# akamiru/bce

Hardware: AMD Instinct MI355X
Metric: MB/s compressed (higher is better)
Workload: dtype u8/u32 integer

## Files before the change

### bce_amd/csrc/host_coder.cpp

```cpp
#include "host_coder.h"

#include "bce_core.h"

#include <stdio.h>
#include <stdlib.h>
#include <string.h>

#include <chrono>
#include <thread>

namespace bce {

const uint8_t kDefaultConfig[9][32] = {
    {0, 0, 5, 5, 5, 4, 4, 4, 4, 4, 4, 4, 4, 4, 4, 4, 4, 4, 4, 4, 4, 4, 4, 4, 4, 4, 4, 4, 4, 4, 4, 0},
    {0, 0, 5, 5, 5, 4, 4, 4, 4, 4, 4, 4, 4, 4, 4, 4, 4, 4, 4, 4, 4, 4, 4, 4, 4, 4, 4, 4, 4, 4, 4, 0},
    {0, 0, 5, 5, 5, 4, 4, 4, 4, 4, 4, 4, 4, 4, 4, 4, 4, 4, 4, 4, 4, 4, 4, 4, 4, 4, 4, 3, 3, 3, 3, 0},
    {0, 0, 5, 5, 5, 4, 4, 4, 4, 4, 4, 4, 4, 4, 4, 4, 4, 4, 4, 4, 4, 4, 3, 3, 3, 3, 3, 3, 3, 3, 3, 0},
    {0, 0, 5, 5, 4, 4, 4, 4, 4, 4, 4, 4, 3, 3, 3, 3, 3, 3, 3, 3, 3, 3, 3, 3, 3, 3, 3, 3, 3, 3, 3, 0},
    {0, 0, 5, 5, 4, 4, 4, 4, 4, 4, 4, 4, 3, 3, 3, 3, 3, 3, 3, 3, 3, 3, 3, 3, 3, 3, 3, 3, 3, 3, 3, 0},
    {0, 0, 5, 4, 4, 4, 4, 4, 4, 3, 3, 3, 3, 3, 3, 3, 3, 3, 3, 3, 3, 3, 3, 3, 3, 3, 3, 3, 3, 3, 3, 0},
    {0, 0, 4, 4, 4, 4, 3, 3, 3, 3, 3, 3, 3, 3, 3, 3, 3, 3, 3, 3, 3, 3, 3, 3, 3, 2, 2, 2, 2, 2, 2, 0},
    {0, 0, 0, 0, 0, 0, 0, 0, 0, 0, 0, 0, 0, 0, 0, 0, 0, 0, 0, 0, 0, 0, 0, 0, 0, 0, 0, 0, 0, 0, 0, 0}};

void RangeCoder::setv(uint32_t s) {
  while (s) { uniform(s & 1, 3); s >>= 1; }
  uniform(2, 3);
}

void RangeCoder::preamble(const uint8_t row[32]) {
  uint32_t last = 0;
  for (int b = 0; b < 32; ++b) {
    const uint32_t bit = row[b];
    uniform(bit != last, 2);
    if (bit != last) uniform(bit, 6);
    last = bit;
  }
}

void RangeCoder::flush() {
  while (!((h_ ^ l_) >> 48)) {
    data_.push_back((uint16_t)(h_ >> 48));
    l_ = (l_ << 16) + 0x0000;
    h_ = (h_ << 16) + 0xFFFF;
  }
  const uint32_t bits = (uint32_t)__builtin_clzll(l_ ^ h_) + 1;
  data_.push_back((uint16_t)((h_ >> (64 - bits)) << (16 - bits)));
}

void HostCoder::begin(const uint8_t config[9][32], const uint32_t C[8], uint32_t n) {
  drain();
  failed_.store(false);
  for (int i = 0; i < 8; ++i) {
    w_[i].busy = 0; w_[i].nsym = 0; w_[i].idle = 0; w_[i].started = false;
    plane[i] = RangeCoder();
    plane[i].preamble(config[i]);
    plane[i].uniform(C[i], n + 1);
  }
}

const Recip *recip_table() {
  static const std::vector<Recip> tab = [] {
    std::vector<Recip> t(kRecipMax);
    t[0] = t[1] = Recip{0, -1, 0};
    for (uint32_t d = 2; d < kRecipMax; ++d) {
      uint32_t L = 0;
      while ((2ull << L) <= d) ++L;
      if ((d & (d - 1)) == 0) { t[d] = Recip{1ull << (64 - L), -1, 0}; continue; }
      const unsigned __int128 two_s = (unsigned __int128)1 << (64 + L);
      const uint64_t m_dn = (uint64_t)(two_s / d);
      const uint64_t e_dn = (uint64_t)(two_s - (unsigned __int128)m_dn * d);
      const uint64_t e_up = d - e_dn;
      if (e_up <= (1ull << L)) t[d] = Recip{m_dn + 1, -1, L};
      else t[d] = Recip{m_dn, 0, L};
    }
    return t;
  }();
  return tab.data();
}

uint64_t bce_test_div_recip(uint64_t x, uint32_t d) {
  return x == ~0ull ? x / d : div_recip1(x + 1, recip_table()[d]);
}

void RangeCoder::encode_run(const uint64_t *out, uint64_t begin, uint64_t end) {
  const Recip *rt = recip_table();
  uint64_t l = l_, R = h_ - l_ + 1;
  uint16_t stage[64];
  uint32_t ns = 0;
#define BCE_EMIT(v)                                                                                       \
  do {                                                                                                    \
    stage[ns++] = (uint16_t)(v);                                                                          \
    if (__builtin_expect(ns == 64, 0)) { data_.insert(data_.end(), stage, stage + 64); ns = 0; }          \
  } while (0)
#define BCE_STEP(cum, freq, total)                                                                        \
  do {                                                                                                    \
    const uint32_t t_ = (total);                                                                          \
    if (__builtin_expect(R - 1 < t_, 0)) {                                                  \
      for (int i_ = 0; i_ < 4; ++i_) BCE_EMIT(l >> (48 - 16 * i_));                                       \
      l = 0; R = 0;                                                                                       \
    }                                                                                                     \
    const uint64_t step_ =                                                                                \
        (__builtin_expect(R == 0, 0) || t_ >= kRecipMax) ? (R - 1) / t_ : div_recip1(R, rt[t_]);          \
    l += step_ * (cum);                                                                         \
    R = step_ * (freq);                                                \
    while (__builtin_expect(!(((l + R - 1) ^ l) >> 48), 0)) {                     \
      BCE_EMIT((l + R - 1) >> 48);                                                                        \
      l <<= 16;                                                                                           \
      R <<= 16;                                                             \
    }                                                                                                     \
  } while (0)
#define BCE_BIT(bit)                                                                                      \
  do {                                                                                                    \
    if (__builtin_expect(R - 1 < 2u, 0)) {                                                  \
      for (int i_ = 0; i_ < 4; ++i_) BCE_EMIT(l >> (48 - 16 * i_));                                       \
      l = 0; R = 0;                                                                                       \
    }                                                                                                     \
    const uint64_t step_ = (R - 1) >> 1;                                                                  \
    l += step_ & (0ull - (uint64_t)(bit));                                                                \
    R = step_;                                                                                            \
    while (__builtin_expect(!(((l + R - 1) ^ l) >> 48), 0)) {                                             \
      BCE_EMIT((l + R - 1) >> 48);                                                                        \
      l <<= 16;                                                                                           \
      R <<= 16;                                                                                           \
    }                                                                                                     \
  } while (0)
  for (uint64_t i = begin; i < end; ++i) {
    const uint64_t o = out[i];
    uint32_t es = out_esc_sentinel(o);
    if (__builtin_expect(es != 1u, 0))
      for (; es > 1u; es >>= 1) BCE_BIT(es & 1u);
    BCE_STEP(out_cum(o), out_freq(o), out_total(o));
  }
#undef BCE_BIT
#undef BCE_STEP
#undef BCE_EMIT
  data_.insert(data_.end(), stage, stage + ns);
  l_ = l; h_ = l + R - 1;
}

void HostCoder::consume(int p, const SymRun *runs, size_t nruns, const uint64_t *out) {
  RangeCoder &rc = plane[p];
  for (size_t r = 0; r < nruns; ++r) rc.encode_run(out, runs[r].start, runs[r].start + runs[r].count);
}

HostCoder::HostCoder() {
  try {
    for (int p = 0; p < 8; ++p) w_[p].th = std::thread([this, p]() { run(p); });
  } catch (...) {
    stop_threads();
    throw;
  }
}

void HostCoder::stop_threads() {
  for (int p = 0; p < 8; ++p) {
    { std::lock_guard<std::mutex> g(w_[p].mu); w_[p].stop = true; }
    w_[p].cv.notify_all();
  }
  for (int p = 0; p < 8; ++p) if (w_[p].th.joinable()) w_[p].th.join();
}

HostCoder::~HostCoder() { stop_threads(); }

void HostCoder::run(int p) {
  Worker &w = w_[p];
  for (;;) {
    CoderBatch *b = nullptr;
    double wait_s = 0;
    {
      std::unique_lock<std::mutex> lk(w.mu);
      const bool dry = w.q.empty();
      const auto tw = std::chrono::steady_clock::now();
      w.cv.wait(lk, [&] { return w.stop || !w.q.empty(); });
      if (w.q.empty()) return;
      b = w.q.front();
      w.q.pop_front();
      wait_s = dry ? std::chrono::duration<double>(std::chrono::steady_clock::now() - tw).count() : 0.0;
    }
    const auto t0 = std::chrono::steady_clock::now();
    try {
      if (b->wait_ready) {
        b->wait_ready();
        wait_s += std::chrono::duration<double>(std::chrono::steady_clock::now() - t0).count();
      }
      if (!failed_.load(std::memory_order_relaxed) && ((plane_mask >> p) & 1u)) {
        consume(p, b->runs[p].data(), b->runs[p].size(), b->out);
        for (const SymRun &r : b->runs[p]) w.nsym += r.count;
      }
    } catch (...) {
      failed_.store(true);
    }
    const double dt = std::chrono::duration<double>(std::chrono::steady_clock::now() - t0).count();
    {
      std::lock_guard<std::mutex> g(done_mu_);
      w.busy += dt;
      if (w.started) w.idle += wait_s;
      w.started = true;
      b->pending.fetch_sub(1);
      ++completed_;
    }
    done_cv_.notify_all();
  }
}

void HostCoder::submit(CoderBatch *b) {
  b->pending.store(8);
  { std::lock_guard<std::mutex> g(done_mu_); submitted_ += 8; }
  for (int p = 0; p < 8; ++p) {
    { std::lock_guard<std::mutex> g(w_[p].mu); w_[p].q.push_back(b); }
    w_[p].cv.notify_one();
  }
}

void HostCoder::wait(CoderBatch *b) {
  std::unique_lock<std::mutex> lk(done_mu_);
  done_cv_.wait(lk, [&] { return b->pending.load() == 0; });
}

void HostCoder::drain() {
  std::unique_lock<std::mutex> lk(done_mu_);
  done_cv_.wait(lk, [&] { return completed_ == submitted_; });
}

double HostCoder::busy_seconds() {
  std::lock_guard<std::mutex> g(done_mu_);
  double m = 0;
  for (int p = 0; p < 8; ++p) m = w_[p].busy > m ? w_[p].busy : m;
  return m;
}

double HostCoder::idle_seconds(int p) {
  std::lock_guard<std::mutex> g(done_mu_);
  return w_[p].idle;
}

void HostCoder::finish(const uint8_t config[9][32], uint32_t n, uint32_t offset) {
  if (getenv("BCE_HIP_CODER_DEBUG"))
    for (int p = 0; p < 8; ++p) fprintf(stderr, "coder %d: busy %.1f ms, %llu symbols, %zu words\n", p, w_[p].busy * 1e3, (unsigned long long)w_[p].nsym, plane[p].data().size());
  for (int i = 0; i < 8; ++i) plane[i].flush();
  rebuild_header(config, n, offset);
}

void HostCoder::rebuild_header(const uint8_t config[9][32], uint32_t n, uint32_t offset) {
  unsigned size = 0u;
  for (int i = 0; i < 8; ++i) size += (unsigned)plane[i].data().size();
  RangeCoder mainc;
  mainc.preamble(config[8]);
  mainc.setv(n);
  mainc.uniform(offset, n + 1);
  mainc.setv(size);
  int s = (int)size;
  for (int i = 0; i < 7; ++i) {
    mainc.uniform((uint32_t)plane[i].data().size(), (uint32_t)s + 1);
    s -= (int)plane[i].data().size();
  }
  mainc.flush();
  header_ = mainc.data();
}

size_t HostCoder::archive_words() const {
  size_t w = 1 + header_.size();
  for (int i = 0; i < 8; ++i) w += plane[i].data().size();
  return w;
}

void HostCoder::assemble(uint16_t *dst) const {
  *dst++ = (uint16_t)header_.size();
  memcpy(dst, header_.data(), header_.size() * 2);
  dst += header_.size();
  uint16_t *at[8];
  for (int i = 0; i < 8; ++i) { at[i] = dst; dst += plane[i].data().size(); }
  size_t total = 0;
  for (int i = 0; i < 8; ++i) total += plane[i].data().size();
  if (total < (1u << 20)) {
    for (int i = 0; i < 8; ++i) memcpy(at[i], plane[i].data().data(), plane[i].data().size() * 2);
    return;
  }
  std::thread th[8];
  int started = 0;
  try {
    for (; started < 8; ++started) {
      const int i = started;
      th[i] = std::thread([this, i, &at] { memcpy(at[i], plane[i].data().data(), plane[i].data().size() * 2); });
    }
  } catch (...) {
  }
  for (int i = started; i < 8; ++i) memcpy(at[i], plane[i].data().data(), plane[i].data().size() * 2);
  for (int i = 0; i < started; ++i) th[i].join();
}

void HostCoder::finish(const uint8_t config[9][32], uint32_t n, uint32_t offset, std::vector<uint16_t> &archive) {
  finish(config, n, offset);
  archive.resize(archive_words());
  assemble(archive.data());
}

}
```

### bce_amd/csrc/host_coder.h

```cpp
#pragma once
#include <stddef.h>
#include <stdint.h>

#include <atomic>
#include <condition_variable>
#include <deque>
#include <functional>
#include <mutex>
#include <thread>
#include <vector>

namespace bce {

class alignas(128) RangeCoder {
 public:
  RangeCoder() : l_(0), h_(~0ull) {}
  inline void encode(uint32_t cum, uint32_t freq, uint32_t total) {
    if (__builtin_expect(h_ - l_ < total, 0)) {
      for (int i = 0; i < 4; ++i) data_.push_back((uint16_t)(l_ >> (48 - 16 * i)));
      l_ = 0; h_ = ~0ull;
    }
    const uint64_t step = (h_ - l_) / total;
    l_ += step * cum;
    h_ = l_ + step * freq - 1;
    while (!((h_ ^ l_) >> 48)) {
      data_.push_back((uint16_t)(h_ >> 48));
      l_ = (l_ << 16) + 0x0000;
      h_ = (h_ << 16) + 0xFFFF;
    }
  }
  inline void uniform(uint32_t s, uint32_t k) { encode(s, 1, k); }
  void setv(uint32_t s);
  void preamble(const uint8_t row[32]);
  void flush();
  const std::vector<uint16_t> &data() const { return data_; }
  std::vector<uint16_t> &data() { return data_; }
  void encode_run(const uint64_t *out, uint64_t begin, uint64_t end);

 private:
  uint64_t l_, h_;
  std::vector<uint16_t> data_;
};

struct SymRun { uint64_t start; uint32_t count; uint32_t round; };

struct CoderBatch {
  const uint64_t *out = nullptr;
  std::function<void()> wait_ready;
  std::vector<SymRun> runs[8];
  std::atomic<int> pending{0};
};

struct HostCoder {
  RangeCoder plane[8];
  uint32_t plane_mask = 0xFFu;
  void set_stream(int p, const uint16_t *words, size_t n) { plane[p].data().assign(words, words + n); }
  void rebuild_header(const uint8_t config[9][32], uint32_t n, uint32_t offset);
  HostCoder();
  ~HostCoder();
  void begin(const uint8_t config[9][32], const uint32_t C[8], uint32_t n);
  void consume(int p, const SymRun *runs, size_t nruns, const uint64_t *out);
  void submit(CoderBatch *b);
  void wait(CoderBatch *b);
  void drain();
  void finish(const uint8_t config[9][32], uint32_t n, uint32_t offset);
  size_t archive_words() const;
  void assemble(uint16_t *dst) const;
  void finish(const uint8_t config[9][32], uint32_t n, uint32_t offset, std::vector<uint16_t> &archive);
  double busy_seconds();
  double idle_seconds(int p);
  bool failed() const { return failed_.load(); }

 private:
  struct Worker {
    std::thread th;
    std::mutex mu;
    std::condition_variable cv;
    std::deque<CoderBatch *> q;
    double busy = 0, idle = 0;
    bool started = false;
    uint64_t nsym = 0;
    bool stop = false;
  };
  Worker w_[8];
  std::mutex done_mu_;
  std::condition_variable done_cv_;
  std::vector<uint16_t> header_;
  uint64_t submitted_ = 0, completed_ = 0;
  std::atomic<bool> failed_{false};
  void run(int p);
  void stop_threads();
};

struct Recip { uint64_t m; int32_t am1; uint32_t sh; };
constexpr uint32_t kRecipMax = 8192;
const Recip *recip_table();
inline uint64_t div_recip1(uint64_t x1, const Recip &r) {
  return (uint64_t)(((unsigned __int128)r.m * (x1 + (uint64_t)(int64_t)r.am1)) >> 64) >> r.sh;
}
inline uint64_t div_small(uint64_t x, uint32_t d, const Recip *rt) {
  return (x == ~0ull || d >= kRecipMax) ? x / d : div_recip1(x + 1, rt[d]);
}

extern const uint8_t kDefaultConfig[9][32];
uint64_t bce_test_div_recip(uint64_t x, uint32_t d);

}
```

Before: 922.0.

## Reuse persistent coder workers for archive assembly copy and align hot encode loop

Archive assembly no longer spawns eight fresh std::threads per call. It hands each persistent coder worker an equal byte slice of the concatenated streams to memcpy, with a small copy flag and a pending counter guarded by the existing done mutex. This spreads the copy evenly across threads instead of one thread per plane, and it removes thread creation cost. The encode_run hot loop is also placed in its own 64-byte-aligned text section, with an optional padding knob. Debug timing instrumentation for the coder tail is added too, at the cost of extra clock reads and more synchronisation state.

```diff
diff --git a/bce_amd/csrc/host_coder.cpp b/bce_amd/csrc/host_coder.cpp
--- a/bce_amd/csrc/host_coder.cpp
+++ b/bce_amd/csrc/host_coder.cpp
@@ -6,6 +6,7 @@
 #include <stdlib.h>
 #include <string.h>
 
+#include <algorithm>
 #include <chrono>
 #include <thread>
 
@@ -47,8 +48,12 @@
   data_.push_back((uint16_t)((h_ >> (64 - bits)) << (16 - bits)));
 }
 
+static double steady_s() { return std::chrono::duration<double>(std::chrono::steady_clock::now().time_since_epoch()).count(); }
+
 void HostCoder::begin(const uint8_t config[9][32], const uint32_t C[8], uint32_t n) {
+  const double t0 = steady_s();
   drain();
+  std::lock_guard<std::mutex> copying(copy_mu_);
   failed_.store(false);
   for (int i = 0; i < 8; ++i) {
     w_[i].busy = 0; w_[i].nsym = 0; w_[i].idle = 0; w_[i].started = false;
@@ -56,6 +61,7 @@
     plane[i].preamble(config[i]);
     plane[i].uniform(C[i], n + 1);
   }
+  t_begin_s_ = steady_s() - t0;
 }
 
 const Recip *recip_table() {
@@ -82,7 +88,18 @@
   return x == ~0ull ? x / d : div_recip1(x + 1, recip_table()[d]);
 }
 
-void RangeCoder::encode_run(const uint64_t *out, uint64_t begin, uint64_t end) {
+#ifdef BCE_CODER_UNPLACED
+#define BCE_HOT_LOOP
+#elif defined(BCE_CODER_PAD)
+#define BCE_STR2(x) #x
+#define BCE_STR(x) BCE_STR2(x)
+__asm__(".pushsection .text.bce_encode_run,\"ax\",@progbits\n.balign 64\n.skip " BCE_STR(BCE_CODER_PAD) ", 0xcc\n.popsection");
+#define BCE_HOT_LOOP __attribute__((section(".text.bce_encode_run"), aligned(16)))
+#else
+#define BCE_HOT_LOOP __attribute__((section(".text.bce_encode_run"), aligned(64)))
+#endif
+
+BCE_HOT_LOOP void RangeCoder::encode_run(const uint64_t *out, uint64_t begin, uint64_t end) {
   const Recip *rt = recip_table();
   uint64_t l = l_, R = h_ - l_ + 1;
   uint16_t stage[64];
@@ -167,15 +184,28 @@
   for (;;) {
     CoderBatch *b = nullptr;
     double wait_s = 0;
+    bool copy = false;
     {
       std::unique_lock<std::mutex> lk(w.mu);
       const bool dry = w.q.empty();
       const auto tw = std::chrono::steady_clock::now();
-      w.cv.wait(lk, [&] { return w.stop || !w.q.empty(); });
-      if (w.q.empty()) return;
-      b = w.q.front();
-      w.q.pop_front();
-      wait_s = dry ? std::chrono::duration<double>(std::chrono::steady_clock::now() - tw).count() : 0.0;
+      w.cv.wait(lk, [&] { return w.stop || w.copy || !w.q.empty(); });
+      if (!w.q.empty()) {
+        b = w.q.front();
+        w.q.pop_front();
+        wait_s = dry ? std::chrono::duration<double>(std::chrono::steady_clock::now() - tw).count() : 0.0;
+      } else if (w.copy) {
+        w.copy = false;
+        copy = true;
+      } else {
+        return;
+      }
+    }
+    if (copy) {
+      copy_streams(copy_dst_, copy_words_ * (size_t)p / 8, copy_words_ * (size_t)(p + 1) / 8);
+      { std::lock_guard<std::mutex> g(done_mu_); --copy_pending_; }
+      done_cv_.notify_all();
+      continue;
     }
     const auto t0 = std::chrono::steady_clock::now();
     try {
@@ -190,9 +220,11 @@
     } catch (...) {
       failed_.store(true);
     }
-    const double dt = std::chrono::duration<double>(std::chrono::steady_clock::now() - t0).count();
+    const auto t1 = std::chrono::steady_clock::now();
+    const double dt = std::chrono::duration<double>(t1 - t0).count();
     {
       std::lock_guard<std::mutex> g(done_mu_);
+      t_batch_done_ = std::max(t_batch_done_, std::chrono::duration<double>(t1.time_since_epoch()).count());
       w.busy += dt;
       if (w.started) w.idle += wait_s;
       w.started = true;
@@ -220,6 +252,7 @@
 void HostCoder::drain() {
   std::unique_lock<std::mutex> lk(done_mu_);
   done_cv_.wait(lk, [&] { return completed_ == submitted_; });
+  t_drained_ = steady_s();
 }
 
 double HostCoder::busy_seconds() {
@@ -237,8 +270,10 @@
 void HostCoder::finish(const uint8_t config[9][32], uint32_t n, uint32_t offset) {
   if (getenv("BCE_HIP_CODER_DEBUG"))
     for (int p = 0; p < 8; ++p) fprintf(stderr, "coder %d: busy %.1f ms, %llu symbols, %zu words\n", p, w_[p].busy * 1e3, (unsigned long long)w_[p].nsym, plane[p].data().size());
+  t_finish0_ = steady_s();
   for (int i = 0; i < 8; ++i) plane[i].flush();
   rebuild_header(config, n, offset);
+  t_finish1_ = steady_s();
 }
 
 void HostCoder::rebuild_header(const uint8_t config[9][32], uint32_t n, uint32_t offset) {
@@ -264,29 +299,52 @@
   return w;
 }
 
-void HostCoder::assemble(uint16_t *dst) const {
+void HostCoder::copy_streams(uint16_t *dst, size_t from, size_t to) const {
+  size_t at = 0;
+  for (int i = 0; i < 8 && at < to; ++i) {
+    const std::vector<uint16_t> &d = plane[i].data();
+    const size_t lo = from > at ? from : at, hi = to < at + d.size() ? to : at + d.size();
+    if (lo < hi) memcpy(dst + lo, d.data() + (lo - at), (hi - lo) * 2);
+    at += d.size();
+  }
+}
+
+bool HostCoder::copy_by_threads(uint16_t *dst, size_t words) {
+  if (failed()) return false;
+  copy_dst_ = dst; copy_words_ = words;
+  { std::lock_guard<std::mutex> g(done_mu_); copy_pending_ = 8; }
+  int handed = 0;
+  for (; handed < 8; ++handed) {
+    Worker &w = w_[handed];
+    std::lock_guard<std::mutex> g(w.mu);
+    if (w.stop) break;
+    w.copy = true;
+  }
+  for (int p = 0; p < handed; ++p) w_[p].cv.notify_one();
+  for (int p = handed; p < 8; ++p) copy_streams(dst, words * (size_t)p / 8, words * (size_t)(p + 1) / 8);
+  std::unique_lock<std::mutex> lk(done_mu_);
+  copy_pending_ -= 8 - handed;
+  done_cv_.wait(lk, [&] { return copy_pending_ == 0; });
+  return true;
+}
+
+void HostCoder::assemble(uint16_t *dst) {
+  const double t0 = steady_s();
+  std::lock_guard<std::mutex> copying(copy_mu_);
   *dst++ = (uint16_t)header_.size();
   memcpy(dst, header_.data(), header_.size() * 2);
   dst += header_.size();
-  uint16_t *at[8];
-  for (int i = 0; i < 8; ++i) { at[i] = dst; dst += plane[i].data().size(); }
   size_t total = 0;
   for (int i = 0; i < 8; ++i) total += plane[i].data().size();
-  if (total < (1u << 20)) {
-    for (int i = 0; i < 8; ++i) memcpy(at[i], plane[i].data().data(), plane[i].data().size() * 2);
-    return;
-  }
-  std::thread th[8];
-  int started = 0;
-  try {
-    for (; started < 8; ++started) {
-      const int i = started;
-      th[i] = std::thread([this, i, &at] { memcpy(at[i], plane[i].data().data(), plane[i].data().size() * 2); });
-    }
-  } catch (...) {
-  }
-  for (int i = started; i < 8; ++i) memcpy(at[i], plane[i].data().data(), plane[i].data().size() * 2);
-  for (int i = 0; i < started; ++i) th[i].join();
+  if (total * 2 < (1u << 20) || !copy_by_threads(dst, total)) copy_streams(dst, 0, total);
+  if (getenv("BCE_HIP_CODER_DEBUG")) {
+    double done, drained;
+    { std::lock_guard<std::mutex> g(done_mu_); done = t_batch_done_; drained = t_drained_; }
+    const double t1 = steady_s();
+    fprintf(stderr, "coder tail: %.3f ms from the last batch coded to the archive laid out (drain woke after %.3f ms, finish %.3f ms, assemble %.3f ms "
+            "of %zu words, the rest between them); begin %.3f ms\n", (t1 - done) * 1e3, (drained - done) * 1e3, (t_finish1_ - t_finish0_) * 1e3,
+            (t1 - t0) * 1e3, total, t_begin_s_ * 1e3);
+  }
 }
 
 void HostCoder::finish(const uint8_t config[9][32], uint32_t n, uint32_t offset, std::vector<uint16_t> &archive) {
diff --git a/bce_amd/csrc/host_coder.h b/bce_amd/csrc/host_coder.h
--- a/bce_amd/csrc/host_coder.h
+++ b/bce_amd/csrc/host_coder.h
@@ -65,7 +65,7 @@
   void drain();
   void finish(const uint8_t config[9][32], uint32_t n, uint32_t offset);
   size_t archive_words() const;
-  void assemble(uint16_t *dst) const;
+  void assemble(uint16_t *dst);
   void finish(const uint8_t config[9][32], uint32_t n, uint32_t offset, std::vector<uint16_t> &archive);
   double busy_seconds();
   double idle_seconds(int p);
@@ -81,6 +81,7 @@
     bool started = false;
     uint64_t nsym = 0;
     bool stop = false;
+    bool copy = false;
   };
   Worker w_[8];
   std::mutex done_mu_;
@@ -88,6 +89,13 @@
   std::vector<uint16_t> header_;
   uint64_t submitted_ = 0, completed_ = 0;
   std::atomic<bool> failed_{false};
+  std::mutex copy_mu_;
+  uint16_t *copy_dst_ = nullptr;
+  size_t copy_words_ = 0;
+  int copy_pending_ = 0;
+  void copy_streams(uint16_t *dst, size_t from, size_t to) const;
+  bool copy_by_threads(uint16_t *dst, size_t words);
+  double t_batch_done_ = 0, t_drained_ = 0, t_finish0_ = 0, t_finish1_ = 0, t_begin_s_ = 0;
   void run(int p);
   void stop_threads();
 };
```

After: 931.9, median of 6. +1.1%, better.
